# BruceGeLi/TCE_RL

Measured on AMD Instinct MI355X. Metric: env-steps/sec (TCE rollout + update, Metaworld-reach-like, 4096 envs/GPU), higher is better.
Workload: dtype f32

## Files before the change

tce_rl_amd/critic_ops.py:

```python
import torch

from . import _lib
from ._lib import call, ptr, sfx, stream

_ACT = {"tanh": 0, "relu": 1, "leaky_relu": 2, "softplus": 3}


def narrow_supported(mlp):
    return (mlp.dtype == torch.float32 and mlp.dim_out == 1
            and list(mlp.hidden_layers) == [128, 128]
            and 1 <= mlp.dim_in <= 40 and mlp.act_func_last_type is None
            and mlp.act_func_hidden_type in _ACT)


def wide_supported(mlp):
    hl = list(mlp.hidden_layers)
    if not (mlp.dim_out == 1 and len(hl) == 2 and hl[0] == hl[1]
            and mlp.act_func_last_type is None
            and mlp.act_func_hidden_type in _ACT
            and mlp.dtype in (torch.float32, torch.float64)):
        return False
    if narrow_supported(mlp):
        return False
    esize = 4 if mlp.dtype == torch.float32 else 8
    return bool(_lib.load().tce_mlpw_supported(mlp.dim_in, hl[0], esize))


def supported(mlp):
    return narrow_supported(mlp) or wide_supported(mlp)


def _rows(x):
    din = x.shape[-1]
    if x.dim() == 3 and x.stride(2) == 1:
        N, T, _ = x.shape
        return x, x.stride(0), x.stride(1), T, N * T
    x2 = x.reshape(-1, din)
    if x2.stride(1) != 1:
        x2 = x2.contiguous()
    return x2, 0, x2.stride(0), x2.shape[0], x2.shape[0]


def _weights(mlp):
    ls = mlp.layers
    return [ptr(t) for t in (ls[0].weight, ls[0].bias, ls[1].weight,
                             ls[1].bias, ls[2].weight, ls[2].bias)]


def forward(mlp, x):
    if wide_supported(mlp):
        return _wide_forward(mlp, x)
    xs, es, rs, T, R = _rows(x)
    out = torch.empty(R, dtype=torch.float32, device=x.device)
    call("tce_mlp_critic_f32", ptr(xs), es, rs, T, R, mlp.dim_in,
         *_weights(mlp), _ACT[mlp.act_func_hidden_type], None, None, 0.0,
         ptr(out), None, None, None, 0, None, None, None, None, 0.0, 0.0, 0.0,
         0.0, 0.0, 0.0, 1.0, None, stream())
    return out.reshape(*x.shape[:-1], 1)


def _wide_ws(mlp, R, backward):
    H = mlp.hidden_layers[0]
    n = _lib.load().tce_mlpw_workspace_len(R, H, int(backward))
    ws = getattr(mlp, "_tce_wide_ws", None)
    dev = mlp.layers[0].weight.device
    if ws is None or ws.numel() < n or ws.dtype != mlp.dtype or ws.device != dev:
        ws = torch.empty(n, dtype=mlp.dtype, device=dev)
        mlp._tce_wide_ws = ws
    return ws


def _wide_forward(mlp, x):
    xs, es, rs, T, R = _rows(x)
    out = torch.empty(R, dtype=mlp.dtype, device=x.device)
    ws = _wide_ws(mlp, R, False)
    call("tce_mlpw_critic_" + sfx(mlp.dtype), ptr(xs), es, rs, T, R,
         mlp.dim_in, mlp.hidden_layers[0], *_weights(mlp),
         _ACT[mlp.act_func_hidden_type], None, None, 0.0, ptr(out), ptr(ws),
         None, None, None, 0, None, None, None, None, 0.0, 0.0, 0.0, 0.0, 0.0,
         0.0, 1.0, None, stream())
    return out.reshape(*x.shape[:-1], 1)


class WideEpochRunner:
    arith = "f32"

    def __init__(self, mlp, flat=None, arith="f32"):
        assert wide_supported(mlp) and arith == "f32"
        self.mlp = mlp
        lib = _lib.load()
        self.H = mlp.hidden_layers[0]
        self.P = lib.tce_mlpw_num_params(mlp.dim_in, self.H)
        dev = mlp.layers[0].weight.device
        if flat is None:
            flat = torch.zeros(self.P, dtype=mlp.dtype, device=dev)
        assert flat.numel() == self.P and flat.dtype == mlp.dtype
        self.flat = flat
        self.entry = "tce_mlpw_critic_" + sfx(mlp.dtype)
        self.partials = torch.empty(lib.tce_mlpw_grid(), self.P + 2,
                                    dtype=mlp.dtype, device=dev)
        off = 0
        self.params = list(mlp.parameters())
        self.views = []
        for p in self.params:
            self.views.append(self.flat[off:off + p.numel()].view_as(p))
            off += p.numel()
        assert off == self.P

    def epoch(self, states, returns, old_values, clip, max_workgroups=0,
              stats=None, adam=None, xchg=None, grad_scale=1.0):
        xs, es, rs, T, R = _rows(states)
        ret = returns.reshape(-1)
        ret = ret if ret.is_contiguous() else ret.contiguous()
        old = old_values.reshape(-1).contiguous() if clip > 0 else None
        if stats is None:
            stats = torch.zeros(4, dtype=self.mlp.dtype,
                                device=self.flat.device)
        if adam is not None:
            g = adam.param_groups[0]
            adam.host_step += 1
            adam._opt_called = True
            ad = (ptr(adam.flat_param), ptr(adam.m), ptr(adam.v),
                  ptr(adam.dev_state), float(g["lr"]), float(g["betas"][0]),
                  float(g["betas"][1]), float(g["eps"]),
                  float(g["weight_decay"]), float(adam.host_step))
        else:
            ad = (None, None, None, None, 0.0, 0.0, 0.0, 0.0, 0.0, 0.0)
        ws = _wide_ws(self.mlp, R, True)
        call(self.entry, ptr(xs), es, rs, T, R, self.mlp.dim_in, self.H,
             *_weights(self.mlp), _ACT[self.mlp.act_func_hidden_type],
             ptr(ret), ptr(old), float(clip), None, ptr(ws),
             ptr(self.partials), ptr(self.flat), ptr(stats),
             int(max_workgroups), *ad, float(grad_scale),
             None if xchg is None else xchg.handle, stream())
        for p, v in zip(self.params, self.views):
            p.grad = v
        return stats


    def epoch_minibatches(self, states, returns, old_values, clip, row_index,
                          num_minibatches, stats, adam, grad_clip=0.0,
                          max_workgroups=0, xchg=None, grad_scale=1.0):
        xs, es, rs, T, R = _rows(states)
        assert row_index.dtype == torch.int64 and row_index.numel() == R \
            and row_index.is_contiguous()
        assert stats.shape == (num_minibatches, 4) and stats.is_contiguous()
        ret = returns.reshape(-1)
        ret = ret if ret.is_contiguous() else ret.contiguous()
        old = old_values.reshape(-1).contiguous() if clip > 0 else None
        g = adam.param_groups[0]
        first = adam.host_step + 1
        adam.host_step += num_minibatches
        adam._opt_called = True
        ws = _wide_ws(self.mlp, -(-R // num_minibatches), True)
        call(self.entry.replace("critic_", "critic_minibatch_"), ptr(xs), es,
             rs, T, R, self.mlp.dim_in, self.H, *_weights(self.mlp),
             _ACT[self.mlp.act_func_hidden_type], ptr(ret), ptr(old),
             float(clip), ptr(row_index), int(num_minibatches), ptr(ws),
             ptr(self.partials), ptr(self.flat), ptr(stats),
             int(max_workgroups), ptr(adam.flat_param), ptr(adam.m),
             ptr(adam.v), ptr(adam.dev_state), float(g["lr"]),
             float(g["betas"][0]), float(g["betas"][1]), float(g["eps"]),
             float(g["weight_decay"]), float(first), float(grad_clip),
             float(grad_scale), None if xchg is None else xchg.handle,
             stream())
        for p, v in zip(self.params, self.views):
            p.grad = v
        return stats


def make_runner(mlp, flat=None, arith="f32"):
    if wide_supported(mlp):
        return WideEpochRunner(mlp, flat, "f32")
    return EpochRunner(mlp, flat, arith)


class EpochRunner:

    def __init__(self, mlp, flat=None, arith="f32"):
        assert narrow_supported(mlp)
        assert arith in ("f32", "f16x2", "bf16x3"), arith
        self.arith = arith
        self.entry = "tce_mlp_critic_" + arith
        self.mlp = mlp
        lib = _lib.load()
        self.P = lib.tce_mlp_critic_num_params(mlp.dim_in)
        dev = mlp.layers[0].weight.device
        if flat is None:
            flat = torch.zeros(self.P, dtype=torch.float32, device=dev)
        assert flat.numel() == self.P and flat.dtype == torch.float32
        self.flat = flat
        self.partials = torch.empty(lib.tce_mlp_critic_grid(), self.P + 2,
                                    dtype=torch.float32, device=dev)
        off = 0
        self.params = list(mlp.parameters())
        self.views = []
        for p in self.params:
            self.views.append(self.flat[off:off + p.numel()].view_as(p))
            off += p.numel()
        assert off == self.P

    def epoch(self, states, returns, old_values, clip, max_workgroups=0,
              stats=None, adam=None, xchg=None, grad_scale=1.0):
        xs, es, rs, T, R = _rows(states)
        ret = returns.reshape(-1)
        ret = ret if ret.is_contiguous() else ret.contiguous()
        old = None
        if clip > 0:
            old = old_values.reshape(-1).contiguous()
        if stats is None:
            stats = torch.zeros(4, dtype=torch.float32, device=self.flat.device)
        if adam is not None:
            g = adam.param_groups[0]
            adam.host_step += 1
            adam._opt_called = True
            ad = (ptr(adam.flat_param), ptr(adam.m), ptr(adam.v),
                  ptr(adam.dev_state), float(g["lr"]), float(g["betas"][0]),
                  float(g["betas"][1]), float(g["eps"]),
                  float(g["weight_decay"]), float(adam.host_step))
        else:
            ad = (None, None, None, None, 0.0, 0.0, 0.0, 0.0, 0.0, 0.0)
        call(self.entry, ptr(xs), es, rs, T, R, self.mlp.dim_in,
             *_weights(self.mlp), _ACT[self.mlp.act_func_hidden_type],
             ptr(ret), ptr(old), float(clip), None, ptr(self.partials),
             ptr(self.flat), ptr(stats), int(max_workgroups), *ad,
             float(grad_scale), None if xchg is None else xchg.handle,
             stream())
        for p, v in zip(self.params, self.views):
            p.grad = v
        return stats


    def epoch_minibatches(self, states, returns, old_values, clip, row_index,
                          num_minibatches, stats, adam, grad_clip=0.0,
                          max_workgroups=0, xchg=None, grad_scale=1.0):
        if self.arith != "f32":
            raise NotImplementedError(
                "minibatched critic epochs run on the exact-fp32 kernel only "
                "(critic_arith=%s)" % self.arith)
        xs, es, rs, T, R = _rows(states)
        assert row_index.dtype == torch.int64 and row_index.numel() == R \
            and row_index.is_contiguous()
        assert stats.shape == (num_minibatches, 4) and stats.is_contiguous()
        ret = returns.reshape(-1)
        ret = ret if ret.is_contiguous() else ret.contiguous()
        old = old_values.reshape(-1).contiguous() if clip > 0 else None
        g = adam.param_groups[0]
        first = adam.host_step + 1
        adam.host_step += num_minibatches
        adam._opt_called = True
        call("tce_mlp_critic_minibatch_f32", ptr(xs), es, rs, T, R,
             self.mlp.dim_in, *_weights(self.mlp),
             _ACT[self.mlp.act_func_hidden_type], ptr(ret), ptr(old),
             float(clip), ptr(row_index), int(num_minibatches),
             ptr(self.partials), ptr(self.flat), ptr(stats),
             int(max_workgroups), ptr(adam.flat_param), ptr(adam.m),
             ptr(adam.v), ptr(adam.dev_state), float(g["lr"]),
             float(g["betas"][0]), float(g["betas"][1]), float(g["eps"]),
             float(g["weight_decay"]), float(first), float(grad_clip),
             float(grad_scale), None if xchg is None else xchg.handle,
             stream())
        for p, v in zip(self.params, self.views):
            p.grad = v
        return stats


def hidden_supported(mlp, x):
    return (mlp.dtype == torch.float32 and list(mlp.hidden_layers) == [128, 128]
            and 1 <= mlp.dim_in <= 40 and mlp.act_func_hidden_type in _ACT
            and x.is_cuda and x.dtype == torch.float32)


class _Hidden2(torch.autograd.Function):

    @staticmethod
    def forward(ctx, x, w1, b1, w2, b2, act):
        xs, es, rs, T, R = _rows(x)
        out = torch.empty(R, 128, dtype=torch.float32, device=x.device)
        call("tce_mlp_hidden_f32", ptr(xs), es, rs, T, R, x.shape[-1], ptr(w1),
             ptr(b1), ptr(w2), ptr(b2), act, None, ptr(out), None, None, None,
             stream())
        ctx.save_for_backward(xs, w1, b1, w2, b2)
        ctx.geom = (es, rs, T, R, x.shape[-1], act)
        return out.reshape(*x.shape[:-1], 128)

    @staticmethod
    def backward(ctx, g):
        xs, w1, b1, w2, b2 = ctx.saved_tensors
        es, rs, T, R, din, act = ctx.geom
        lib = _lib.load()
        P = lib.tce_mlp_critic_num_params(din)
        dev = g.device
        g = g.reshape(R, 128)
        g = g if g.is_contiguous() else g.contiguous()
        partials = torch.empty(min(lib.tce_mlp_critic_grid(), (R + 63) // 64),
                               P + 2, dtype=torch.float32, device=dev)
        grad = torch.empty(P, dtype=torch.float32, device=dev)
        stats = torch.zeros(2, dtype=torch.float32, device=dev)
        call("tce_mlp_hidden_f32", ptr(xs), es, rs, T, R, din, ptr(w1), ptr(b1),
             ptr(w2), ptr(b2), act, ptr(g), None, ptr(partials), ptr(grad),
             ptr(stats), stream())
        o1, o2, o3 = 128 * din, 128 * din + 128, 128 * din + 128 + 128 * 128
        return (None, grad[:o1].view(128, din), grad[o1:o2],
                grad[o2:o3].view(128, 128), grad[o3:o3 + 128], None)


def hidden_forward(mlp, x):
    ls = mlp.layers
    return _Hidden2.apply(x, ls[0].weight, ls[0].bias, ls[1].weight,
                          ls[1].bias, _ACT[mlp.act_func_hidden_type])
```

tce_rl_amd/csrc/mlp.hip:

```cpp
#include "mlp_shared.h"

extern "C" int tce_xchg_adam_f32(void* xchg, float* param, float* grad, float* m, float* v,
                                 int64_t n, float* state, float* norms_out, float step, float lr,
                                 float beta1, float beta2, float eps, float weight_decay,
                                 float clip, float grad_scale, void* stream);
extern "C" int tce_adam_once_f32(float* param, const float* grad, float* m, float* v, int64_t n,
                                 float* state, float* norms_out, float step, float lr,
                                 float beta1, float beta2, float eps, float weight_decay,
                                 float clip, float grad_scale, void* stream);

namespace {

__device__ inline f32x4 mfma(float a, float b, f32x4 c) {
  return __builtin_amdgcn_mfma_f32_16x16x4f32(a, b, c, 0, 0, 0);
}
__device__ inline void fence_sched() { __builtin_amdgcn_sched_barrier(0); }

__host__ __device__ inline int u1_of(int q) {
  const int kb = q >> 4, r = q & 15;
  return 64 * (kb >> 2) + 16 * (r & 3) + 4 * (r >> 2) + (kb & 3);
}

template <int KPGE>
struct Lds {
  static constexpr int W1P = 4 * KPGE + 2;
  float *W2s, *W1s, *Bs, *Th1, *Tdy;
  __device__ explicit Lds(char* raw) {
    W2s = reinterpret_cast<float*>(raw);
    W1s = W2s + HID * W2P;
    Bs = W1s + HID * W1P;
    Th1 = Bs + 3 * HID;
    Tdy = Th1 + ROWS_PER_TILE * TPT;
  }
};

template <int KPGE>
__device__ inline void stage_weights(const MlpArgs& a, const Lds<KPGE>& L, int tid, int nthreads) {
  constexpr int W1P = Lds<KPGE>::W1P;
  const int din = a.din;
  if ((reinterpret_cast<uintptr_t>(a.w2) & 15) == 0) {
    const f32x4* w2v = reinterpret_cast<const f32x4*>(a.w2);
    constexpr int NV = HID * HID / 4, BATCH = 8;
    for (int e0 = tid; e0 < NV; e0 += BATCH * nthreads) {
      f32x4 v[BATCH];
#pragma unroll
      for (int b = 0; b < BATCH; ++b) {
        const int e = e0 + b * nthreads;
        v[b] = w2v[e < NV ? e : NV - 1];
      }
#pragma unroll
      for (int b = 0; b < BATCH; ++b) {
        const int e = e0 + b * nthreads;
        if (e < NV) *reinterpret_cast<f32x4*>(L.W2s + (e >> 5) * W2P + 4 * (e & 31)) = v[b];
      }
    }
  } else {
    for (int e = tid; e < HID * HID; e += nthreads) L.W2s[(e >> 7) * W2P + (e & 127)] = a.w2[e];
  }
  {
    constexpr int NW1 = HID * 4 * KPGE, BATCH = 8;
    for (int e0 = tid; e0 < NW1; e0 += BATCH * nthreads) {
      float v[BATCH];
#pragma unroll
      for (int b = 0; b < BATCH; ++b) {
        const int e = e0 + b * nthreads < NW1 ? e0 + b * nthreads : NW1 - 1;
        const int q = e / (4 * KPGE), f = e - q * 4 * KPGE;
        v[b] = a.w1[u1_of(q) * din + (f < din ? f : din - 1)];
      }
#pragma unroll
      for (int b = 0; b < BATCH; ++b) {
        const int e = e0 + b * nthreads;
        if (e < NW1) {
          const int q = e / (4 * KPGE), f = e - q * 4 * KPGE;
          L.W1s[q * W1P + f] = f < din ? v[b] : 0.f;
        }
      }
    }
  }
  for (int e = tid; e < HID; e += nthreads) {
    L.Bs[e] = a.b1[u1_of(e)];
    L.Bs[HID + e] = a.b2[e];
    L.Bs[2 * HID + e] = a.w3 ? a.w3[e] : 0.f;
  }
}

template <int KPGE>
__device__ inline int64_t load_x(const MlpArgs& a, const RowCursor& cur, int g, float* dst) {
  const bool in = cur.r < a.R;
  int64_t ne = in ? cur.ne : cur.last_ne;
  int t = in ? cur.t : cur.last_t;
  int64_t phys = in ? cur.r : a.R - 1;
  if (a.row_index) {
    phys = a.row_index[phys];
    ne = phys / a.T;
    t = (int)(phys - ne * a.T);
  }
  const float* xr = a.x + ne * a.env_stride + t * a.row_stride;
#pragma unroll
  for (int s = 0; s < KPGE; ++s) {
    const int k = KPGE * g + s;
    dst[s] = xr[k < a.din ? k : a.din - 1];
  }
  return phys;
}

template <int ACT, int KPGE, bool BIAS_LAST = false>
__device__ inline void forward_chain(const Lds<KPGE>& L, const float* xb, int c, int g,
                                     f32x4* h1, f32x4* h2) {
  constexpr int W1P = Lds<KPGE>::W1P;
  {
    float A[2][2 * KPGE];
    auto ld = [&](int mp, float* d) {
      const float* p = L.W1s + (32 * mp + c) * W1P + KPGE * g;
#pragma unroll
      for (int s = 0; s < KPGE; s += 2) {
        const f32x2 v0 = *reinterpret_cast<const f32x2*>(p + s);
        const f32x2 v1 = *reinterpret_cast<const f32x2*>(p + 16 * W1P + s);
        d[s] = v0.x; d[s + 1] = v0.y;
        d[KPGE + s] = v1.x; d[KPGE + s + 1] = v1.y;
      }
    };
    ld(0, A[0]);
#pragma unroll
    for (int mp = 0; mp < NB / 2; ++mp) {
      if (mp + 1 < NB / 2) ld(mp + 1, A[(mp + 1) & 1]);
      const f32x4 bl0 = *reinterpret_cast<const f32x4*>(L.Bs + 32 * mp + 4 * g);
      const f32x4 bl1 = *reinterpret_cast<const f32x4*>(L.Bs + 32 * mp + 16 + 4 * g);
      const f32x4 zero4 = {0, 0, 0, 0};
      f32x4 acc0 = BIAS_LAST ? zero4 : bl0, acc1 = BIAS_LAST ? zero4 : bl1;
      const f32x4 bias0 = BIAS_LAST ? bl0 : zero4, bias1 = BIAS_LAST ? bl1 : zero4;
      fence_sched();
#pragma unroll
      for (int s = 0; s < KPGE; ++s) {
        acc0 = mfma(A[mp & 1][s], xb[s], acc0);
        acc1 = mfma(A[mp & 1][KPGE + s], xb[s], acc1);
      }
#pragma unroll
      for (int i = 0; i < 4; ++i) {
        acc0[i] = act_f<ACT>(BIAS_LAST ? acc0[i] + bias0[i] : acc0[i]);
        acc1[i] = act_f<ACT>(BIAS_LAST ? acc1[i] + bias1[i] : acc1[i]);
      }
      h1[2 * mp] = acc0;
      h1[2 * mp + 1] = acc1;
    }
  }
  {
    f32x4 A[2][4];
    const float* wb = L.W2s + c * W2P + 4 * g;
    auto ld = [&](int st, f32x4* d) {
      const float* p = wb + (32 * (st >> 2)) * W2P + 16 * (st & 3);
      d[0] = *reinterpret_cast<const f32x4*>(p);
      d[1] = *reinterpret_cast<const f32x4*>(p + 64);
      d[2] = *reinterpret_cast<const f32x4*>(p + 16 * W2P);
      d[3] = *reinterpret_cast<const f32x4*>(p + 16 * W2P + 64);
    };
    ld(0, A[0]);
    f32x4 acc0, acc1, bias0 = {0, 0, 0, 0}, bias1 = {0, 0, 0, 0};
#pragma unroll
    for (int st = 0; st < 16; ++st) {
      const int mp = st >> 2, j = st & 3;
      if (st + 1 < 16) ld(st + 1, A[(st + 1) & 1]);
      if (j == 0) {
        const f32x4 bl0 = *reinterpret_cast<const f32x4*>(L.Bs + HID + 32 * mp + 4 * g);
        const f32x4 bl1 = *reinterpret_cast<const f32x4*>(L.Bs + HID + 32 * mp + 16 + 4 * g);
        if (BIAS_LAST) {
          bias0 = bl0;
          bias1 = bl1;
          acc0 = (f32x4){0, 0, 0, 0};
          acc1 = (f32x4){0, 0, 0, 0};
        } else {
          acc0 = bl0;
          acc1 = bl1;
        }
      }
      fence_sched();
#pragma unroll
      for (int kb = 0; kb < NB; ++kb) {
        acc0 = mfma(A[st & 1][kb >> 2][kb & 3], h1[kb][j], acc0);
        acc1 = mfma(A[st & 1][2 + (kb >> 2)][kb & 3], h1[kb][j], acc1);
      }
      if (j == 3) {
#pragma unroll
        for (int i = 0; i < 4; ++i) {
          acc0[i] = act_f<ACT>(BIAS_LAST ? acc0[i] + bias0[i] : acc0[i]);
          acc1[i] = act_f<ACT>(BIAS_LAST ? acc1[i] + bias1[i] : acc1[i]);
        }
        h2[2 * mp] = acc0;
        h2[2 * mp + 1] = acc1;
      }
    }
  }
}

template <int KPGE>
__device__ inline float value_head(const Lds<KPGE>& L, int g, const f32x4* h2) {
  float v = 0.f;
#pragma unroll
  for (int m = 0; m < NB; ++m) {
    const f32x4 w3v = *reinterpret_cast<const f32x4*>(L.Bs + 2 * HID + 16 * m + 4 * g);
#pragma unroll
    for (int i = 0; i < 4; ++i) v += w3v[i] * h2[m][i];
  }
  return sum_lane_groups(v);
}

template <int ACT, int KPGE>
__global__ __launch_bounds__(MLP_BT, 1) void mlp_critic_fwd_kernel(MlpArgs a) {
  extern __shared__ __attribute__((aligned(16))) char smem_raw[];
  const Lds<KPGE> L(smem_raw);
  const int tid = threadIdx.x;
  const int lane = tid & 63, wave = tid >> 6;
  const int c = lane & 15, g = lane >> 4;
  stage_weights<KPGE>(a, L, tid, MLP_BT);
  __syncthreads();
  const float b3 = a.hout ? 0.f : a.b3[0];
  const int64_t ntiles = (a.R + ROWS_PER_TILE - 1) / ROWS_PER_TILE;
  RowCursor cur(a, blockIdx.x, wave, c);
  float xn[KPGE];
  load_x<KPGE>(a, cur, g, xn);
  for (int64_t tile = blockIdx.x; tile < ntiles; tile += gridDim.x) {
    const int64_t r = cur.r;
    const bool rok = r < a.R;
    float xb[KPGE];
#pragma unroll
    for (int s = 0; s < KPGE; ++s) xb[s] = (KPGE * g + s < a.din && rok) ? xn[s] : 0.f;
    cur.advance(a.T);
    load_x<KPGE>(a, cur, g, xn);
    f32x4 h1[NB], h2[NB];
    forward_chain<ACT, KPGE, true>(L, xb, c, g, h1, h2);
    if (a.hout) {
      if (rok) {
        float* dst = a.hout + r * HID + 4 * g;
#pragma unroll
        for (int m = 0; m < NB; ++m) *reinterpret_cast<f32x4*>(dst + 16 * m) = h2[m];
      }
    } else {
      const float v = value_head<KPGE>(L, g, h2) + b3;
      if (rok && g == 0) a.values[r] = v;
    }
  }
}

template <int ACT, int KPGE, bool HIDDEN>
__global__ __launch_bounds__(2 * MLP_BT, 1) void mlp_critic_bwd_kernel(MlpArgs a) {
  constexpr int NCB = (4 * KPGE + 1 + 15) / 16;
  extern __shared__ __attribute__((aligned(16))) char smem_raw[];
  const Lds<KPGE> L(smem_raw);
  float* Th1 = L.Th1;
  float* Tdy = L.Tdy;
  const int din = a.din;
  const int tid = threadIdx.x;
  const int lane = tid & 63;
  const int role = tid >> 8;
  const int wave = (tid >> 6) & 3;
  const int c = lane & 15, g = lane >> 4;
  stage_weights<KPGE>(a, L, tid, 2 * MLP_BT);
  __syncthreads();
  const int64_t ntiles = (a.R + ROWS_PER_TILE - 1) / ROWS_PER_TILE;
  const int P = mlp_num_params(din);
  float* out = a.partials + (int64_t)blockIdx.x * (P + 2);
  float* oW1 = out;
  float* ob1 = oW1 + HID * din;
  float* oW2 = ob1 + HID;
  float* ob2 = oW2 + HID * HID;
  float* ow3 = ob2 + HID;
  float* ob3 = ow3 + HID;
  __shared__ float sc[8];
  float* red = Th1;

  if (role == 0) {
    const float b3 = HIDDEN ? 0.f : a.b3[0];
    const float inv_n = 1.f / (float)a.R;
    float gw3[NB][4];
#pragma unroll
    for (int m = 0; m < NB; ++m)
#pragma unroll
      for (int i = 0; i < 4; ++i) gw3[m][i] = 0.f;
    float gb3 = 0.f, loss_sum = 0.f;
    float* trow_h = Th1 + (wave * 16 + c) * TPT + 4 * g;
    float* trow_d = Tdy + (wave * 16 + c) * TPT + 4 * g;
    RowCursor cur(a, blockIdx.x, wave, c);
    float xn[KPGE], retn, oldn = 0.f;
    {
      const int64_t rcn = load_x<KPGE>(a, cur, g, xn);
      retn = HIDDEN ? 0.f : a.ret[rcn];
      if (!HIDDEN && a.clip > 0.f) oldn = a.old_v[rcn];
    }
#ifdef MLPX_STAMP
    long long stt[10] = {0, 0, 0, 0, 0, 0, 0, 0, 0, 0};
    long long tprev = __builtin_readcyclecounter();
#define STAMP(k) { const long long tn = __builtin_readcyclecounter(); stt[k] += tn - tprev; tprev = tn; }
#else
#define STAMP(k)
#endif
    for (int64_t tile = blockIdx.x; tile < ntiles; tile += gridDim.x) {
      STAMP(9)
      const int64_t r = cur.r;
      const bool rok = r < a.R;
      float xb[KPGE];
#pragma unroll
      for (int s = 0; s < KPGE; ++s) xb[s] = (KPGE * g + s < din && rok) ? xn[s] : 0.f;
      const float rt = retn, ov = oldn;
      {
        cur.advance(a.T);
        const int64_t rcn = load_x<KPGE>(a, cur, g, xn);
        if (!HIDDEN) {
          retn = a.ret[rcn];
          if (a.clip > 0.f) oldn = a.old_v[rcn];
        }
      }
      f32x4 h1[NB], h2[NB];
      forward_chain<ACT, KPGE>(L, xb, c, g, h1, h2);
      STAMP(0)
      if (HIDDEN) {
        const float* src = a.gh + (rok ? r : a.R - 1) * HID + 4 * g;
#pragma unroll
        for (int m = 0; m < NB; ++m) {
          const f32x4 gv = *reinterpret_cast<const f32x4*>(src + 16 * m);
#pragma unroll
          for (int i = 0; i < 4; ++i)
            h2[m][i] = rok ? gv[i] * act_d<ACT>(h2[m][i]) : 0.f;
        }
      } else {
        const float v = value_head<KPGE>(L, g, h2) + b3;
        if (a.values && rok && g == 0) a.values[r] = v;
        float dv;
        {
          const float e = v - rt;
          float l = e * e, d = 2.f * e;
          if (a.clip > 0.f) {
            const float dlt = v - ov;
            const float cl = fminf(fmaxf(dlt, -a.clip), a.clip);
            const float e2 = ov + cl - rt;
            if (e2 * e2 > l) { l = e2 * e2; d = (dlt > -a.clip && dlt < a.clip) ? 2.f * e2 : 0.f; }
          }
          if (!rok) { l = 0.f; d = 0.f; }
          dv = d * inv_n;
          if (g == 0) loss_sum += l;
          if (g == 0) gb3 += dv;
        }
  #pragma unroll
        for (int m = 0; m < NB; ++m) {
          const f32x4 w3v = *reinterpret_cast<const f32x4*>(L.Bs + 2 * HID + 16 * m + 4 * g);
  #pragma unroll
          for (int i = 0; i < 4; ++i) {
            const float hv = h2[m][i];
            gw3[m][i] += dv * hv;
            h2[m][i] = dv * w3v[i] * act_d<ACT>(hv);
          }
        }
      }
      STAMP(1)
      __syncthreads();
      STAMP(2)
#pragma unroll
      for (int m = 0; m < NB; ++m) {
        *reinterpret_cast<f32x4*>(trow_d + 16 * m) = h2[m];
        *reinterpret_cast<f32x4*>(trow_h + 16 * m) = h1[m];
      }
      __syncthreads();
      STAMP(3)
      f32x4 d1[NB];
      {
#pragma unroll
        for (int kb = 0; kb < NB; ++kb) d1[kb] = (f32x4){0, 0, 0, 0};
        f32x4 A[2][2];
        const float* wb = L.W2s + (4 * g) * W2P + 16 * (c & 3) + 4 * (c >> 2);
        auto ld = [&](int st, f32x4* d) {
          const float* p = wb + (16 * (st >> 2) + (st & 3)) * W2P;
          d[0] = *reinterpret_cast<const f32x4*>(p);
          d[1] = *reinterpret_cast<const f32x4*>(p + 64);
        };
        ld(0, A[0]);
#pragma unroll
        for (int st = 0; st < 32; ++st) {
          if (st + 1 < 32) ld(st + 1, A[(st + 1) & 1]);
          fence_sched();
          const float b = h2[st >> 2][st & 3];
#pragma unroll
#ifndef MLPX_NOB2
          for (int kb = 0; kb < NB; ++kb) d1[kb] = mfma(A[st & 1][kb >> 2][kb & 3], b, d1[kb]);
#else
          for (int kb = 0; kb < 1; ++kb) d1[st & 7][0] += A[st & 1][0][0] * b + A[st & 1][1][1];
#endif
        }
      }
      STAMP(4)
#pragma unroll
      for (int kb = 0; kb < NB; ++kb)
#pragma unroll
        for (int i = 0; i < 4; ++i) d1[kb][i] *= act_d<ACT>(h1[kb][i]);
      STAMP(5)
      __syncthreads();
      STAMP(6)
#pragma unroll
      for (int kb = 0; kb < NB; ++kb) *reinterpret_cast<f32x4*>(trow_d + 16 * kb) = d1[kb];
      {
        float* xs = Th1 + (wave * 16 + c) * XP;
#pragma unroll
        for (int s = 0; s < KPGE; ++s) {
          const int f = KPGE * g + s;
          xs[4 * (f & 15) + (f >> 4)] = xb[s];
        }
        if (g == 0) xs[4 * (din & 15) + (din >> 4)] = rok ? 1.f : 0.f;
      }
      __syncthreads();
      STAMP(7)
    }
    __syncthreads();
#pragma unroll
    for (int m = 0; m < NB; ++m)
#pragma unroll
      for (int i = 0; i < 4; ++i) {
        float v3 = gw3[m][i];
#pragma unroll
        for (int off = 8; off > 0; off >>= 1) v3 += __shfl_xor(v3, off, 16);
        if (c == 0) red[(16 * m + 4 * g + i) * 4 + wave] = v3;
      }
    float s3 = (g == 0) ? gb3 : 0.f, sl = (g == 0) ? loss_sum : 0.f;
    s3 = wave_sum(s3);
    sl = wave_sum(sl);
    if (lane == 0) { sc[wave] = s3; sc[4 + wave] = sl; }
    __syncthreads();
    if (tid < HID) ow3[tid] = (red[tid * 4] + red[tid * 4 + 1]) + (red[tid * 4 + 2] + red[tid * 4 + 3]);
    if (tid == 0) {
      ob3[0] = sc[0] + sc[1] + sc[2] + sc[3];
      ob3[1] = sc[4] + sc[5] + sc[6] + sc[7];
      ob3[2] = 0.f;
    }
#ifdef MLPX_STAMP
    __syncthreads();
    if (tid == 0 && blockIdx.x == 0)
      for (int k = 0; k < 10; ++k) out[k] = (float)stt[k];
#endif
  } else {
    f32x4 gW2[2][NB];
    f32x4 gW1[2][NCB];
    float gb2[2] = {0.f, 0.f};
#pragma unroll
    for (int rb = 0; rb < 2; ++rb) {
#pragma unroll
      for (int n = 0; n < NB; ++n) gW2[rb][n] = (f32x4){0, 0, 0, 0};
#pragma unroll
      for (int n = 0; n < NCB; ++n) gW1[rb][n] = (f32x4){0, 0, 0, 0};
    }
    auto dw1 = [&]() {
      f32x2 av[3];
      f32x4 bv[3];
      auto ld = [&](int t, int buf) {
        const int bt = 4 * t + g;
        av[buf] = *reinterpret_cast<const f32x2*>(Tdy + bt * TPT + 32 * wave + 2 * c);
        bv[buf] = *reinterpret_cast<const f32x4*>(Th1 + bt * XP + 4 * c);
      };
      ld(0, 0);
      ld(1, 1);
#pragma unroll
      for (int t = 0; t < 16; ++t) {
        if (t + 2 < 16) ld(t + 2, (t + 2) % 3);
        fence_sched();
#pragma unroll
#ifndef MLPX_NODW1
        for (int n = 0; n < NCB; ++n) {
          gW1[0][n] = mfma(av[t % 3].x, bv[t % 3][n], gW1[0][n]);
          gW1[1][n] = mfma(av[t % 3].y, bv[t % 3][n], gW1[1][n]);
        }
#else
        for (int n = 0; n < 1; ++n) gW1[0][0][0] += av[t % 3].x * bv[t % 3][0];
#endif
      }
    };
    bool first = true;
#ifdef MLPX_STAMP
    long long gst[4] = {0, 0, 0, 0};
#define GSTAMP(k, t0) gst[k] += __builtin_readcyclecounter() - (t0);
#else
#define GSTAMP(k, t0)
#endif
    for (int64_t tile = blockIdx.x; tile < ntiles; tile += gridDim.x) {
#ifdef MLPX_STAMP
      const long long tg0 = __builtin_readcyclecounter();
#endif
      if (!first) dw1();
      first = false;
      GSTAMP(0, tg0)
      __syncthreads();
      GSTAMP(1, tg0)
      __syncthreads();
#ifdef MLPX_STAMP
      const long long tg1 = __builtin_readcyclecounter();
#endif
      {
        f32x2 av[2];
        f32x4 bv[2][2];
        auto ld = [&](int t, int buf) {
          const int bt = 4 * t + g;
          av[buf] = *reinterpret_cast<const f32x2*>(Tdy + bt * TPT + 32 * wave + 2 * c);
          const float* p = Th1 + bt * TPT + 8 * c;
          bv[buf][0] = *reinterpret_cast<const f32x4*>(p);
          bv[buf][1] = *reinterpret_cast<const f32x4*>(p + 4);
        };
        ld(0, 0);
#pragma unroll
        for (int t = 0; t < 16; ++t) {
          if (t + 1 < 16) ld(t + 1, (t + 1) & 1);
          fence_sched();
          gb2[0] += av[t & 1].x;
          gb2[1] += av[t & 1].y;
#pragma unroll
#ifndef MLPX_NODW2
          for (int n = 0; n < NB; ++n) {
            const float b = bv[t & 1][n >> 2][n & 3];
            gW2[0][n] = mfma(av[t & 1].x, b, gW2[0][n]);
            gW2[1][n] = mfma(av[t & 1].y, b, gW2[1][n]);
          }
#else
          for (int n = 0; n < 1; ++n) gW2[0][t & 7][0] += bv[t & 1][0][0] + bv[t & 1][1][1];
#endif
        }
      }
      GSTAMP(2, tg1)
      __syncthreads();
      GSTAMP(3, tg1)
      __syncthreads();
    }
    if (!first) dw1();
    __syncthreads();
#pragma unroll
    for (int rb = 0; rb < 2; ++rb) {
#pragma unroll
      for (int i = 0; i < 4; ++i) {
        const int qa = 32 * wave + 2 * (4 * g + i) + rb;
#pragma unroll
        for (int n = 0; n < NB; ++n) oW2[qa * HID + u1_of(8 * c + n)] = gW2[rb][n][i];
        const int h = u1_of(qa);
#pragma unroll
        for (int n = 0; n < NCB; ++n) {
          const int f = 16 * n + c;
          if (f < din) oW1[h * din + f] = gW1[rb][n][i];
          else if (f == din) ob1[h] = gW1[rb][n][i];
        }
      }
      float v2 = gb2[rb];
      v2 += __shfl_xor(v2, 16, 64);
      v2 += __shfl_xor(v2, 32, 64);
      if (g == 0) ob2[32 * wave + 2 * c + rb] = v2;
    }
    __syncthreads();
#ifdef MLPX_STAMP
    __syncthreads();
    if (tid == 256 && blockIdx.x == 0)
      for (int k = 0; k < 4; ++k) out[10 + k] = (float)gst[k];
#endif
  }
}

template <int KPGE>
constexpr size_t mlp_lds_bytes(bool bwd = true) {
  return sizeof(float) * ((size_t)HID * W2P + (size_t)HID * (4 * KPGE + 2) + 3 * HID +
                          (bwd ? 2 * (size_t)ROWS_PER_TILE * TPT : 0));
}

template <int ACT, bool BWD, int KPGE>
void mlp_launch(const MlpArgs& a, int grid, hipStream_t st) {
  constexpr size_t lds = mlp_lds_bytes<KPGE>();
  static_assert(lds <= 160 * 1024, "LDS budget");
  if (BWD && a.gh != nullptr) {
    tce_lds_limit(reinterpret_cast<const void*>(mlp_critic_bwd_kernel<ACT, KPGE, true>), (size_t)(lds));
    hipLaunchKernelGGL((mlp_critic_bwd_kernel<ACT, KPGE, true>), dim3(grid), dim3(2 * MLP_BT), lds,
                       st, a);
  } else if (BWD) {
    tce_lds_limit(reinterpret_cast<const void*>(mlp_critic_bwd_kernel<ACT, KPGE, false>), (size_t)(lds));
    hipLaunchKernelGGL((mlp_critic_bwd_kernel<ACT, KPGE, false>), dim3(grid), dim3(2 * MLP_BT), lds,
                       st, a);
  } else {
    constexpr size_t ldsf = mlp_lds_bytes<KPGE>(false);
    tce_lds_limit(reinterpret_cast<const void*>(mlp_critic_fwd_kernel<ACT, KPGE>), (size_t)(ldsf));
    hipLaunchKernelGGL((mlp_critic_fwd_kernel<ACT, KPGE>), dim3(grid), dim3(MLP_BT), ldsf, st, a);
  }
}

template <int ACT>
void mlp_go(bool bwd, const MlpArgs& a, int grid, hipStream_t st) {
  if (a.din <= 24) {
    if (bwd) mlp_launch<ACT, true, 6>(a, grid, st); else mlp_launch<ACT, false, 6>(a, grid, st);
  } else {
    if (bwd) mlp_launch<ACT, true, 10>(a, grid, st); else mlp_launch<ACT, false, 10>(a, grid, st);
  }
}

}

extern "C" int tce_cu_budget_value(void);

extern "C" {

int tce_mlp_critic_hidden(void) { return HID; }
int tce_mlp_critic_grid(void) { return 256; }
int64_t tce_mlp_critic_num_params(int din) { return mlp_num_params(din); }

static int mlp_critic_impl(const float* x, int64_t env_stride, int64_t row_stride, int T,
                           int64_t R, int din, const float* w1, const float* b1,
                           const float* w2, const float* b2, const float* w3, const float* b3,
                           int act, const float* returns, const float* old_values, float clip,
                           float* values, float* partials, float* grad, float* stats,
                           int max_workgroups, float* adam_param, float* adam_m, float* adam_v,
                           float* adam_state, float lr, float beta1, float beta2, float eps,
                           float weight_decay, float adam_step, float grad_scale, void* xchg,
                           void* stream, const int64_t* row_index) {
  TCE_CHECK_ARG(x && w1 && b1 && w2 && b2 && w3 && b3 && R > 0 && T > 0,
                "mlp_critic: null buffer / bad sizes");
  TCE_CHECK_ARG(din >= 1 && din <= MAX_DIN, "mlp_critic: 1 <= D_in <= 40");
  TCE_CHECK_ARG(act >= 0 && act <= 3, "mlp_critic: unknown activation");
  const bool bwd = partials != nullptr;
  TCE_CHECK_ARG(!bwd || (returns && grad && stats), "mlp_critic: backward buffers missing");
  TCE_CHECK_ARG(bwd || values, "mlp_critic: nothing to compute");
  TCE_CHECK_ARG(!(bwd && clip > 0.f && !old_values), "mlp_critic: old values missing");
  TCE_CHECK_ARG(!adam_param || (bwd && adam_m && adam_v && adam_state && adam_step >= 1.f),
                "mlp_critic: fused Adam needs the backward pass and its state buffers");
  TCE_CHECK_ARG(!row_index || (bwd && !values),
                "mlp_critic: a row index goes with the backward pass only (no values output)");
  MlpArgs a{x, env_stride, row_stride, T, R, din, w1, b1, w2, b2, w3, b3,
            returns, old_values, clip, values, partials, nullptr, nullptr, row_index};
  hipStream_t st = (hipStream_t)stream;
  const int64_t ntiles = ceil_div(R, ROWS_PER_TILE);
  int cap = tce_mlp_critic_grid();
  if (max_workgroups > 0 && max_workgroups < cap) cap = max_workgroups;
  const int grid = (int)tmin<int64_t>(cap, ntiles);
  switch (act) {
    case 0: mlp_go<ACT_TANH>(bwd, a, grid, st); break;
    case 1: mlp_go<ACT_RELU>(bwd, a, grid, st); break;
    case 2: mlp_go<ACT_LEAKY>(bwd, a, grid, st); break;
    default: mlp_go<ACT_SOFTPLUS>(bwd, a, grid, st); break;
  }
  TCE_LAUNCH_CHECK();
  if (bwd) {
    const int P = mlp_num_params(din);
    TCE_CHECK_ARG(!xchg || adam_param, "mlp_critic: an exchange needs the fused Adam step");
    AdamArgs ad{xchg ? nullptr : adam_param, adam_m, adam_v, adam_state, lr, beta1, beta2, eps,
                weight_decay, adam_step};
    hipLaunchKernelGGL(mlp_finish_kernel, dim3((unsigned)ceil_div(P + 1, 64)),
                       dim3(64 * FIN_GROUPS), 0, st, partials, grid, P, R, grad, stats, ad);
    TCE_LAUNCH_CHECK();
    if (xchg)
      return tce_xchg_adam_f32(xchg, adam_param, grad, adam_m, adam_v, P, adam_state, stats + 2,
                               adam_step, lr, beta1, beta2, eps, weight_decay, 0.f, grad_scale,
                               stream);
  }
  return 0;
}

int tce_mlp_critic_f32(const float* x, int64_t env_stride, int64_t row_stride, int T,
                       int64_t R, int din, const float* w1, const float* b1,
                       const float* w2, const float* b2, const float* w3, const float* b3,
                       int act, const float* returns, const float* old_values, float clip,
                       float* values, float* partials, float* grad, float* stats,
                       int max_workgroups, float* adam_param, float* adam_m, float* adam_v,
                       float* adam_state, float lr, float beta1, float beta2, float eps,
                       float weight_decay, float adam_step, float grad_scale, void* xchg,
                       void* stream) {
  return mlp_critic_impl(x, env_stride, row_stride, T, R, din, w1, b1, w2, b2, w3, b3, act,
                         returns, old_values, clip, values, partials, grad, stats,
                         max_workgroups, adam_param, adam_m, adam_v, adam_state, lr, beta1, beta2,
                         eps, weight_decay, adam_step, grad_scale, xchg, stream, nullptr);
}

int tce_mlp_critic_minibatch_f32(
    const float* x, int64_t env_stride, int64_t row_stride, int T, int64_t R, int din,
    const float* w1, const float* b1, const float* w2, const float* b2, const float* w3,
    const float* b3, int act, const float* returns, const float* old_values, float clip,
    const int64_t* row_index, int num_minibatches, float* partials, float* grad, float* stats,
    int max_workgroups, float* adam_param, float* adam_m, float* adam_v, float* adam_state,
    float lr, float beta1, float beta2, float eps, float weight_decay, float adam_step,
    float grad_clip, float grad_scale, void* xchg, void* stream) {
  TCE_CHECK_ARG(row_index && num_minibatches >= 1 && R >= num_minibatches,
                "mlp_critic_minibatch: row index missing / more minibatches than rows");
  TCE_CHECK_ARG(adam_param && adam_m && adam_v && adam_state && partials && grad && stats,
                "mlp_critic_minibatch: optimizer / gradient buffers missing");
  const int P = mlp_num_params(din);
  TCE_CHECK_ARG(!(grad_clip > 0.f) || P <= (1 << 17),
                "mlp_critic_minibatch: clipping needs num_params <= 2^17");
  const bool fused = !(grad_clip > 0.f);
  const int64_t base = R / num_minibatches, extra = R % num_minibatches;
  int64_t off = 0;
  for (int mb = 0; mb < num_minibatches; ++mb) {
    const int64_t len = base + (mb < extra ? 1 : 0);
    float* st4 = stats + 4 * mb;
    const float step = adam_step + (float)mb;
    int rc = mlp_critic_impl(x, env_stride, row_stride, T, len, din, w1, b1, w2, b2, w3, b3, act,
                             returns, old_values, clip, nullptr, partials, grad, st4,
                             max_workgroups, fused ? adam_param : nullptr, adam_m, adam_v,
                             adam_state, lr, beta1, beta2, eps, weight_decay, step, grad_scale,
                             fused ? xchg : nullptr, stream, row_index + off);
    if (rc) return rc;
    if (!fused) {
      rc = xchg ? tce_xchg_adam_f32(xchg, adam_param, grad, adam_m, adam_v, P, adam_state,
                                    st4 + 2, step, lr, beta1, beta2, eps, weight_decay,
                                    grad_clip, grad_scale, stream)
                : tce_adam_once_f32(adam_param, grad, adam_m, adam_v, P, adam_state, st4 + 2,
                                    step, lr, beta1, beta2, eps, weight_decay, grad_clip,
                                    grad_scale, stream);
      if (rc) return rc;
    }
    off += len;
  }
  return 0;
}


int tce_mlp_hidden_f32(const float* x, int64_t env_stride, int64_t row_stride, int T,
                       int64_t R, int din, const float* w1, const float* b1,
                       const float* w2, const float* b2, int act, const float* grad_hidden,
                       float* hidden_out, float* partials, float* grad, float* stats,
                       void* stream) {
  TCE_CHECK_ARG(x && w1 && b1 && w2 && b2 && R > 0 && T > 0, "mlp_hidden: null buffer / bad sizes");
  TCE_CHECK_ARG(din >= 1 && din <= MAX_DIN, "mlp_hidden: 1 <= D_in <= 40");
  TCE_CHECK_ARG(act >= 0 && act <= 3, "mlp_hidden: unknown activation");
  const bool bwd = grad_hidden != nullptr;
  TCE_CHECK_ARG(bwd ? (partials && grad && stats) : (hidden_out != nullptr),
                "mlp_hidden: output buffers missing");
  MlpArgs a{x, env_stride, row_stride, T, R, din, w1, b1, w2, b2, nullptr, nullptr,
            nullptr, nullptr, 0.f, nullptr, bwd ? partials : nullptr,
            bwd ? nullptr : hidden_out, grad_hidden};
  hipStream_t st = (hipStream_t)stream;
  const int64_t ntiles = ceil_div(R, ROWS_PER_TILE);
  int grid = (int)tmin<int64_t>(tce_mlp_critic_grid(), ntiles);
#ifndef MLP_HIDDEN_IGNORE_BUDGET
  const int budget = tce_cu_budget_value();
  if (budget > 0 && grid > budget) grid = budget;
#endif
  switch (act) {
    case 0: mlp_go<ACT_TANH>(bwd, a, grid, st); break;
    case 1: mlp_go<ACT_RELU>(bwd, a, grid, st); break;
    case 2: mlp_go<ACT_LEAKY>(bwd, a, grid, st); break;
    default: mlp_go<ACT_SOFTPLUS>(bwd, a, grid, st); break;
  }
  TCE_LAUNCH_CHECK();
  if (bwd) {
    const int P = mlp_num_params(din);
    AdamArgs ad = adam_args_none();
    hipLaunchKernelGGL(mlp_finish_kernel, dim3((unsigned)ceil_div(P + 1, 64)),
                       dim3(64 * FIN_GROUPS), 0, st, partials, grid, P, R, grad, stats, ad);
    TCE_LAUNCH_CHECK();
  }
  return 0;
}

}
```

Baseline: 19.11 million.

## Software-pipeline critic backward kernel across tiles, overlapping forward with backprop

Restructures the critic training kernel's producer loop into a one-tile-deep software pipeline. Each iteration runs the forward chain for the next tile while doing layer-2 backprop for the previous tile, which is read back from LDS. The x-row reload and the gradient-consumer waves' dW2/dW1 phases are rescheduled so the consumer works on the previous tile between barriers. The Python wrapper gains optional values output and a row-count override. The goal is to hide latency and barrier stalls, at the cost of more complex synchronization and register pressure.

```diff
diff --git a/tce_rl_amd/critic_ops.py b/tce_rl_amd/critic_ops.py
--- a/tce_rl_amd/critic_ops.py
+++ b/tce_rl_amd/critic_ops.py
@@ -201,8 +201,15 @@
         assert off == self.P
 
     def epoch(self, states, returns, old_values, clip, max_workgroups=0,
-              stats=None, adam=None, xchg=None, grad_scale=1.0):
+              stats=None, adam=None, xchg=None, grad_scale=1.0, values=None,
+              rows=None):
         xs, es, rs, T, R = _rows(states)
+        if rows is not None:
+            assert 1 <= rows <= R
+            R = int(rows)
+        assert values is None or (self.arith == "f32" and values.is_contiguous()
+                                  and values.dtype == torch.float32
+                                  and values.numel() == R)
         ret = returns.reshape(-1)
         ret = ret if ret.is_contiguous() else ret.contiguous()
         old = None
@@ -222,7 +229,7 @@
             ad = (None, None, None, None, 0.0, 0.0, 0.0, 0.0, 0.0, 0.0)
         call(self.entry, ptr(xs), es, rs, T, R, self.mlp.dim_in,
              *_weights(self.mlp), _ACT[self.mlp.act_func_hidden_type],
-             ptr(ret), ptr(old), float(clip), None, ptr(self.partials),
+             ptr(ret), ptr(old), float(clip), ptr(values), ptr(self.partials),
              ptr(self.flat), ptr(stats), int(max_workgroups), *ad,
              float(grad_scale), None if xchg is None else xchg.handle,
              stream())
diff --git a/tce_rl_amd/csrc/mlp.hip b/tce_rl_amd/csrc/mlp.hip
--- a/tce_rl_amd/csrc/mlp.hip
+++ b/tce_rl_amd/csrc/mlp.hip
@@ -15,6 +15,9 @@
   return __builtin_amdgcn_mfma_f32_16x16x4f32(a, b, c, 0, 0, 0);
 }
 __device__ inline void fence_sched() { __builtin_amdgcn_sched_barrier(0); }
+
+__device__ inline int opaque_s(int v) { asm volatile("" : "+s"(v)); return v; }
+__device__ inline int opaque_v(int v) { asm volatile("" : "+v"(v)); return v; }
 
 __host__ __device__ inline int u1_of(int q) {
   const int kb = q >> 4, r = q & 15;
@@ -85,7 +88,9 @@
 }
 
 template <int KPGE>
-__device__ inline int64_t load_x(const MlpArgs& a, const RowCursor& cur, int g, float* dst) {
+__device__ inline int64_t load_x(const MlpArgs& a, const RowCursor& cur, int g, float* dst,
+                                 const float** row = nullptr, int din = -1) {
+  if (din < 0) din = a.din;
   const bool in = cur.r < a.R;
   int64_t ne = in ? cur.ne : cur.last_ne;
   int t = in ? cur.t : cur.last_t;
@@ -99,8 +104,9 @@
 #pragma unroll
   for (int s = 0; s < KPGE; ++s) {
     const int k = KPGE * g + s;
-    dst[s] = xr[k < a.din ? k : a.din - 1];
-  }
+    dst[s] = xr[k < din ? k : din - 1];
+  }
+  if (row) *row = xr;
   return phys;
 }
 
@@ -268,6 +274,11 @@
   __shared__ float sc[8];
   float* red = Th1;
 
+#ifdef MLPX_PRIO
+  if ((__builtin_amdgcn_readfirstlane(threadIdx.x) >= 256) == (MLPX_PRIO == 2))
+    __builtin_amdgcn_s_setprio(1);
+#endif
+
   if (role == 0) {
     const float b3 = HIDDEN ? 0.f : a.b3[0];
     const float inv_n = 1.f / (float)a.R;
@@ -281,8 +292,9 @@
     float* trow_d = Tdy + (wave * 16 + c) * TPT + 4 * g;
     RowCursor cur(a, blockIdx.x, wave, c);
     float xn[KPGE], retn, oldn = 0.f;
+    const float *xrn, *xr = nullptr;
     {
-      const int64_t rcn = load_x<KPGE>(a, cur, g, xn);
+      const int64_t rcn = load_x<KPGE>(a, cur, g, xn, &xrn);
       retn = HIDDEN ? 0.f : a.ret[rcn];
       if (!HIDDEN && a.clip > 0.f) oldn = a.old_v[rcn];
     }
@@ -293,90 +305,40 @@
 #else
 #define STAMP(k)
 #endif
-    for (int64_t tile = blockIdx.x; tile < ntiles; tile += gridDim.x) {
+    bool rok = false, have = false;
+    for (int64_t tile = blockIdx.x; have || tile < ntiles; tile += gridDim.x) {
       STAMP(9)
-      const int64_t r = cur.r;
-      const bool rok = r < a.R;
+      const bool next = tile < ntiles;
+      const int64_t r1 = cur.r;
+      const bool rok1 = next && r1 < a.R;
+      f32x4 h1[NB], h2[NB];
+      const float* xr1 = xrn;
+#pragma unroll
+      for (int s = 0; s < KPGE; ++s) xn[s] = (KPGE * g + s < din && rok1) ? xn[s] : 0.f;
+      if (next) forward_chain<ACT, KPGE>(L, xn, opaque_v(c), opaque_v(g), h1, h2);
+      STAMP(0)
+      f32x4 d1[NB];
       float xb[KPGE];
-#pragma unroll
-      for (int s = 0; s < KPGE; ++s) xb[s] = (KPGE * g + s < din && rok) ? xn[s] : 0.f;
-      const float rt = retn, ov = oldn;
-      {
-        cur.advance(a.T);
-        const int64_t rcn = load_x<KPGE>(a, cur, g, xn);
-        if (!HIDDEN) {
-          retn = a.ret[rcn];
-          if (a.clip > 0.f) oldn = a.old_v[rcn];
-        }
-      }
-      f32x4 h1[NB], h2[NB];
-      forward_chain<ACT, KPGE>(L, xb, c, g, h1, h2);
-      STAMP(0)
-      if (HIDDEN) {
-        const float* src = a.gh + (rok ? r : a.R - 1) * HID + 4 * g;
-#pragma unroll
-        for (int m = 0; m < NB; ++m) {
-          const f32x4 gv = *reinterpret_cast<const f32x4*>(src + 16 * m);
-#pragma unroll
-          for (int i = 0; i < 4; ++i)
-            h2[m][i] = rok ? gv[i] * act_d<ACT>(h2[m][i]) : 0.f;
-        }
-      } else {
-        const float v = value_head<KPGE>(L, g, h2) + b3;
-        if (a.values && rok && g == 0) a.values[r] = v;
-        float dv;
-        {
-          const float e = v - rt;
-          float l = e * e, d = 2.f * e;
-          if (a.clip > 0.f) {
-            const float dlt = v - ov;
-            const float cl = fminf(fmaxf(dlt, -a.clip), a.clip);
-            const float e2 = ov + cl - rt;
-            if (e2 * e2 > l) { l = e2 * e2; d = (dlt > -a.clip && dlt < a.clip) ? 2.f * e2 : 0.f; }
-          }
-          if (!rok) { l = 0.f; d = 0.f; }
-          dv = d * inv_n;
-          if (g == 0) loss_sum += l;
-          if (g == 0) gb3 += dv;
-        }
-  #pragma unroll
-        for (int m = 0; m < NB; ++m) {
-          const f32x4 w3v = *reinterpret_cast<const f32x4*>(L.Bs + 2 * HID + 16 * m + 4 * g);
-  #pragma unroll
-          for (int i = 0; i < 4; ++i) {
-            const float hv = h2[m][i];
-            gw3[m][i] += dv * hv;
-            h2[m][i] = dv * w3v[i] * act_d<ACT>(hv);
-          }
-        }
-      }
-      STAMP(1)
-      __syncthreads();
-      STAMP(2)
-#pragma unroll
-      for (int m = 0; m < NB; ++m) {
-        *reinterpret_cast<f32x4*>(trow_d + 16 * m) = h2[m];
-        *reinterpret_cast<f32x4*>(trow_h + 16 * m) = h1[m];
-      }
-      __syncthreads();
-      STAMP(3)
-      f32x4 d1[NB];
-      {
+      if (have) {
 #pragma unroll
         for (int kb = 0; kb < NB; ++kb) d1[kb] = (f32x4){0, 0, 0, 0};
-        f32x4 A[2][2];
-        const float* wb = L.W2s + (4 * g) * W2P + 16 * (c & 3) + 4 * (c >> 2);
+        f32x4 A[2][2], B[2];
+        const int cq = opaque_v(c);
+        const float* wb = L.W2s + (4 * opaque_v(g)) * W2P + 16 * (cq & 3) + 4 * (cq >> 2);
         auto ld = [&](int st, f32x4* d) {
           const float* p = wb + (16 * (st >> 2) + (st & 3)) * W2P;
           d[0] = *reinterpret_cast<const f32x4*>(p);
           d[1] = *reinterpret_cast<const f32x4*>(p + 64);
         };
         ld(0, A[0]);
+        B[0] = *reinterpret_cast<const f32x4*>(trow_d);
 #pragma unroll
         for (int st = 0; st < 32; ++st) {
           if (st + 1 < 32) ld(st + 1, A[(st + 1) & 1]);
+          if ((st & 3) == 0 && st + 4 < 32)
+            B[((st >> 2) + 1) & 1] = *reinterpret_cast<const f32x4*>(trow_d + 16 * ((st >> 2) + 1));
           fence_sched();
-          const float b = h2[st >> 2][st & 3];
+          const float b = B[(st >> 2) & 1][st & 3];
 #pragma unroll
 #ifndef MLPX_NOB2
           for (int kb = 0; kb < NB; ++kb) d1[kb] = mfma(A[st & 1][kb >> 2][kb & 3], b, d1[kb]);
@@ -384,30 +346,103 @@
           for (int kb = 0; kb < 1; ++kb) d1[st & 7][0] += A[st & 1][0][0] * b + A[st & 1][1][1];
 #endif
         }
-      }
+        fence_sched();
+        const int dq = opaque_s(din);
+#pragma unroll
+        for (int s = 0; s < KPGE; ++s) {
+          const int k = KPGE * g + s;
+          xb[s] = xr[k < dq ? k : dq - 1];
+        }
+#pragma unroll
+        for (int kb = 0; kb < NB; ++kb) {
+          const f32x4 hv = *reinterpret_cast<const f32x4*>(trow_h + 16 * kb);
+#pragma unroll
+          for (int i = 0; i < 4; ++i) d1[kb][i] *= act_d<ACT>(hv[i]);
+        }
+      }
+      STAMP(1)
+      __syncthreads();
+      STAMP(2)
+      if (have) {
+#pragma unroll
+        for (int kb = 0; kb < NB; ++kb) *reinterpret_cast<f32x4*>(trow_d + 16 * kb) = d1[kb];
+        float* xs = Th1 + (wave * 16 + c) * XP;
+        const int gq = opaque_v(g);
+#pragma unroll
+        for (int s = 0; s < KPGE; ++s) {
+          const int f = KPGE * gq + s;
+          xs[4 * (f & 15) + (f >> 4)] = (f < din && rok) ? xb[s] : 0.f;
+        }
+        if (g == 0) xs[4 * (din & 15) + (din >> 4)] = rok ? 1.f : 0.f;
+      }
+      STAMP(3)
+      __syncthreads();
       STAMP(4)
-#pragma unroll
-      for (int kb = 0; kb < NB; ++kb)
-#pragma unroll
-        for (int i = 0; i < 4; ++i) d1[kb][i] *= act_d<ACT>(h1[kb][i]);
+      if (next) {
+        if (HIDDEN) {
+          const float* src = a.gh + (rok1 ? r1 : a.R - 1) * HID + 4 * g;
+#pragma unroll
+          for (int m = 0; m < NB; ++m) {
+            const f32x4 gv = *reinterpret_cast<const f32x4*>(src + 16 * m);
+#pragma unroll
+            for (int i = 0; i < 4; ++i)
+              h2[m][i] = rok1 ? gv[i] * act_d<ACT>(h2[m][i]) : 0.f;
+          }
+        } else {
+          const float rt = retn, ov = oldn;
+          const int gq = opaque_v(g);
+          const float v = value_head<KPGE>(L, gq, h2) + b3;
+          if (a.values && rok1 && g == 0) a.values[r1] = v;
+          float dv;
+          {
+            const float e = v - rt;
+            float l = e * e, d = 2.f * e;
+            if (a.clip > 0.f) {
+              const float dlt = v - ov;
+              const float cl = fminf(fmaxf(dlt, -a.clip), a.clip);
+              const float e2 = ov + cl - rt;
+              if (e2 * e2 > l) { l = e2 * e2; d = (dlt > -a.clip && dlt < a.clip) ? 2.f * e2 : 0.f; }
+            }
+            if (!rok1) { l = 0.f; d = 0.f; }
+            dv = d * inv_n;
+            if (g == 0) loss_sum += l;
+            if (g == 0) gb3 += dv;
+          }
+#pragma unroll
+          for (int m = 0; m < NB; ++m) {
+            const f32x4 w3v = *reinterpret_cast<const f32x4*>(L.Bs + 2 * HID + 16 * m + 4 * gq);
+#pragma unroll
+            for (int i = 0; i < 4; ++i) {
+              const float hv = h2[m][i];
+              gw3[m][i] += dv * hv;
+              h2[m][i] = dv * w3v[i] * act_d<ACT>(hv);
+            }
+          }
+        }
+        xr = xr1;
+        cur.advance(a.T);
+        const int64_t rcn = load_x<KPGE>(a, cur, g, xn, &xrn, opaque_s(din));
+        if (!HIDDEN) {
+          retn = a.ret[rcn];
+          if (a.clip > 0.f) oldn = a.old_v[rcn];
+        }
+      }
+      rok = rok1;
+      have = next;
       STAMP(5)
       __syncthreads();
       STAMP(6)
-#pragma unroll
-      for (int kb = 0; kb < NB; ++kb) *reinterpret_cast<f32x4*>(trow_d + 16 * kb) = d1[kb];
-      {
-        float* xs = Th1 + (wave * 16 + c) * XP;
-#pragma unroll
-        for (int s = 0; s < KPGE; ++s) {
-          const int f = KPGE * g + s;
-          xs[4 * (f & 15) + (f >> 4)] = xb[s];
-        }
-        if (g == 0) xs[4 * (din & 15) + (din >> 4)] = rok ? 1.f : 0.f;
-      }
+      if (next) {
+#pragma unroll
+        for (int m = 0; m < NB; ++m) {
+          *reinterpret_cast<f32x4*>(trow_d + 16 * m) = h2[m];
+          *reinterpret_cast<f32x4*>(trow_h + 16 * m) = h1[m];
+        }
+      }
+      STAMP(7)
       __syncthreads();
-      STAMP(7)
-    }
-    __syncthreads();
+      STAMP(8)
+    }
 #pragma unroll
     for (int m = 0; m < NB; ++m)
 #pragma unroll
@@ -469,62 +504,58 @@
 #endif
       }
     };
-    bool first = true;
+    auto dw2 = [&]() {
+      f32x2 av[2];
+      f32x4 bv[2][2];
+      auto ld = [&](int t, int buf) {
+        const int bt = 4 * t + g;
+        av[buf] = *reinterpret_cast<const f32x2*>(Tdy + bt * TPT + 32 * wave + 2 * c);
+        const float* p = Th1 + bt * TPT + 8 * c;
+        bv[buf][0] = *reinterpret_cast<const f32x4*>(p);
+        bv[buf][1] = *reinterpret_cast<const f32x4*>(p + 4);
+      };
+      ld(0, 0);
+#pragma unroll
+      for (int t = 0; t < 16; ++t) {
+        if (t + 1 < 16) ld(t + 1, (t + 1) & 1);
+        fence_sched();
+        gb2[0] += av[t & 1].x;
+        gb2[1] += av[t & 1].y;
+#pragma unroll
+#ifndef MLPX_NODW2
+        for (int n = 0; n < NB; ++n) {
+          const float b = bv[t & 1][n >> 2][n & 3];
+          gW2[0][n] = mfma(av[t & 1].x, b, gW2[0][n]);
+          gW2[1][n] = mfma(av[t & 1].y, b, gW2[1][n]);
+        }
+#else
+        for (int n = 0; n < 1; ++n) gW2[0][t & 7][0] += bv[t & 1][0][0] + bv[t & 1][1][1];
+#endif
+      }
+    };
 #ifdef MLPX_STAMP
-    long long gst[4] = {0, 0, 0, 0};
-#define GSTAMP(k, t0) gst[k] += __builtin_readcyclecounter() - (t0);
+    long long gst[6] = {0, 0, 0, 0, 0, 0};
+    long long gprev = __builtin_readcyclecounter();
+#define GSTAMP(k) { const long long tn = __builtin_readcyclecounter(); gst[k] += tn - gprev; gprev = tn; }
 #else
-#define GSTAMP(k, t0)
-#endif
-    for (int64_t tile = blockIdx.x; tile < ntiles; tile += gridDim.x) {
-#ifdef MLPX_STAMP
-      const long long tg0 = __builtin_readcyclecounter();
-#endif
-      if (!first) dw1();
-      first = false;
-      GSTAMP(0, tg0)
+#define GSTAMP(k)
+#endif
+    bool have = false;
+    for (int64_t tile = blockIdx.x; have || tile < ntiles; tile += gridDim.x) {
+      GSTAMP(5)
+      if (have) dw2();
+      GSTAMP(0)
       __syncthreads();
-      GSTAMP(1, tg0)
+      GSTAMP(1)
       __syncthreads();
-#ifdef MLPX_STAMP
-      const long long tg1 = __builtin_readcyclecounter();
-#endif
-      {
-        f32x2 av[2];
-        f32x4 bv[2][2];
-        auto ld = [&](int t, int buf) {
-          const int bt = 4 * t + g;
-          av[buf] = *reinterpret_cast<const f32x2*>(Tdy + bt * TPT + 32 * wave + 2 * c);
-          const float* p = Th1 + bt * TPT + 8 * c;
-          bv[buf][0] = *reinterpret_cast<const f32x4*>(p);
-          bv[buf][1] = *reinterpret_cast<const f32x4*>(p + 4);
-        };
-        ld(0, 0);
-#pragma unroll
-        for (int t = 0; t < 16; ++t) {
-          if (t + 1 < 16) ld(t + 1, (t + 1) & 1);
-          fence_sched();
-          gb2[0] += av[t & 1].x;
-          gb2[1] += av[t & 1].y;
-#pragma unroll
-#ifndef MLPX_NODW2
-          for (int n = 0; n < NB; ++n) {
-            const float b = bv[t & 1][n >> 2][n & 3];
-            gW2[0][n] = mfma(av[t & 1].x, b, gW2[0][n]);
-            gW2[1][n] = mfma(av[t & 1].y, b, gW2[1][n]);
-          }
-#else
-          for (int n = 0; n < 1; ++n) gW2[0][t & 7][0] += bv[t & 1][0][0] + bv[t & 1][1][1];
-#endif
-        }
-      }
-      GSTAMP(2, tg1)
+      GSTAMP(2)
+      if (have) dw1();
+      GSTAMP(3)
       __syncthreads();
-      GSTAMP(3, tg1)
+      GSTAMP(4)
       __syncthreads();
-    }
-    if (!first) dw1();
-    __syncthreads();
+      have = tile < ntiles;
+    }
 #pragma unroll
     for (int rb = 0; rb < 2; ++rb) {
 #pragma unroll
@@ -549,7 +580,7 @@
 #ifdef MLPX_STAMP
     __syncthreads();
     if (tid == 256 && blockIdx.x == 0)
-      for (int k = 0; k < 4; ++k) out[10 + k] = (float)gst[k];
+      for (int k = 0; k < 6; ++k) out[10 + k] = (float)gst[k];
 #endif
   }
 }
```

Result: no change. 18.93 million (-1.0%).
